# LSDOlab/femo_alpha

Measured on AMD Instinct MI355X. Metric: DOF/s (assembly+solve), forward solve of the RM shell; adjoint-gradient wallclock in adjoint_ms, higher is better.
Workload: dtype f64

## Files before the change

### femo_alpha_amd/csrc/femo_hip.hip

```cpp
#include "../../include/femo_hip.h"
#include "shell_device.h"
#include "frontal.h"
#include "sweeps_multi.h"
#include "shape_sens.h"
#include "residual_jvp.h"
#include "stress.h"
#include "stress_grad.h"
#include "stress_history.h"
#include "disp_history.h"
#include "ply_failure.h"
#include "field_jvp.h"
#include "layup.h"
#include "csr_map.h"
#include "hip_handles.h"

#include <hip/hip_runtime.h>

#include <algorithm>
#include <cmath>
#include <cstdio>
#include <cstdlib>
#include <cstring>
#include <string>
#include <utility>
// ... 5 lines not shown
constexpr int WIDE_CNT_DEFAULT = 512;

#define FEMO_VERSION 101

static std::string g_create_error;

struct femo_ctx {
    int device = 0;
    Stream stream;
    int krylov = 0;
    DevBuf<double> bi[5];
    int tab_nq = 0;
    double hK_mean = 0;
    DevBuf<double> mr_v, mr_y, mr_work, mr_scal;
    PinnedBuf<double> mr_scal_host;
    DevBuf<double> mr_io;
    long long opt_version = 0;
    Stream stream2;
    Event ev_la[2];
    Event ev_sp[2];
    Stream stream_g;
    Event ev_g[2];
    Stream stream_m;
    Event ev_da[2];
    Stream stream3;
    Stream stream_a;
    Event ev_a[3];
    Event ev_x[2];
    int nn = 0, nel = 0, nvc = 0, npc = 0, nP2 = 0, ndof_u = 0, ndof = 0, ld = 0;
    int nghost = 0;
// ... 102 lines not shown
        int fuse_rows_np = 2 * NBO;
        int sweep_graph = 0;
        int diag_v1_cnt = 512;
        int split_cnt = 0, split_groups = 2;
        int super_tiles = 0, super_tiles_min = 8;
        int diag_ahead = 0;
        int fused_schur = 1;
        int equilibrate = 0;
        int precond_nquad = 0;
        int grid_chunk = 32768;
        int wide_np = WIDE_NP_DEFAULT, wide_cnt = WIDE_CNT_DEFAULT;
        int strict = 1;
        int allow_pivot_repair = 0;
        int profile_verbose = 0;
        int big_tiles = 0, big_min_wg = 512;
        int strip_cnt = 0, strip_kmax = STRIP_KMAX, strip_depth = 1;
        int diag_v1 = 0;
        int swork_slots = 8192;
        int xinv_small_cnt = 32;
        int bnd_tiled_nb = 1 << 30;
        int sweep_butterfly = 3;
        int sweep_fuse = 0;
        int sweep_w = 0;
        int assemble_fc = 1;
        int sweep_ahead = 2;
        int apply_lanes = 0;
        int diag_t = 0;
        int multi_rhs = 1;
        int stale_factor = 0;
        double stale_rel = 2e-3;
        int sweep_read_mode = 0;
        int sh_levels_per_thread = 0;
        int sh_chunk = 0;
        int dh_chunk = 0;
// ... 626 lines not shown
            const dim3 grid(nt * (nt + 1) / 2, cnt);
            { ProfScope ps(c, 3);
              FOR_FRONT_CHUNKS(cnt, off, n)
                  hipLaunchKernelGGL(k_extend_gather, dim3(grid.x, n), dim3(256), 0, c->stream, fd, lev, off, mask, fused_schur ? 1 : 0); }
        }
        const bool wide = fr.h_level_wide[L];
        const int cnt_level = cnt, max_np_level = max_np;
        const int* lev_level = lev;
        const bool level_right = c->opt.trailing == 2 ? true : c->opt.trailing == 1 ? false : (cnt_level < c->opt.left_min || cnt_level > c->opt.left_max);
        const bool level_sp = level_right && SP_opt > NBO && cnt_level <= c->opt.super_panel_cnt && max_np_level > NBO;
        const bool level_la = level_right && !level_sp && cnt_level < c->opt.lookahead_cnt && c->opt.lookahead != 0;
        const bool split = wide && c->stream_g && cnt_level >= 2 && cnt_level <= c->opt.split_cnt && !level_la &&
                           !(level_sp && (c->opt.super_panel_ahead || c->opt.diag_ahead));
        const int ngroups = split ? std::max(2, std::min(cnt_level, c->opt.split_groups)) : 1;
        const int chunk_cap = split ? (cnt_level + ngroups - 1) / ngroups : wide ? cnt_level : std::min(cnt_level, fr.swork_slots);
        if (split) {
            HIPCHK(c, hipEventRecord(c->ev_g[0], c->stream));
            HIPCHK(c, hipStreamWaitEvent(c->stream_g, c->ev_g[0], 0));
        }
        for (int chunk_b = b; chunk_b < fr.h_level_off[L + 1]; chunk_b += chunk_cap) {
        hipStream_t st = (split && ((chunk_b - fr.h_level_off[L]) / chunk_cap) % 2 == 1) ? c->stream_g : c->stream;
        const int b = chunk_b, e = std::min(chunk_b + chunk_cap, fr.h_level_off[L + 1]);
        const int cnt = e - b;
        const int* lev = fr.level_nodes + b;
        int max_np = 0;
        for (int i = b; i < e; ++i) max_np = std::max(max_np, fr.h_npiv[fr.h_level_nodes[i]]);
        int max_nf = 0;
        for (int i = b; i < e; ++i) max_nf = std::max(max_nf, fr.h_nf[fr.h_level_nodes[i]]);
        int max_nb = 0;
        for (int i = b; i < e; ++i) max_nb = std::max(max_nb, fr.h_nf[fr.h_level_nodes[i]] - fr.h_npiv[fr.h_level_nodes[i]]);
        const bool right_looking = c->opt.trailing == 2 ? true : c->opt.trailing == 1 ? false : (cnt_level < c->opt.left_min || cnt_level > c->opt.left_max);
        const bool use_sp = right_looking && SP_opt > NBO && cnt_level <= c->opt.super_panel_cnt && max_np_level > NBO;
        const bool lookahead = right_looking && !use_sp && cnt_level < c->opt.lookahead_cnt && c->opt.lookahead != 0;
        bool bulk_pending = false;
        auto count_trailing = [&](int C0, int schur, int K0 = 0, int KW = NBO) {
            if (!fr.profile) return;
            double fl = 0, by = 0;
            for (int i = b; i < e; ++i) {
                const int t = fr.h_level_nodes[i], np = fr.h_npiv[t], nf = fr.h_nf[t];
                const TrailRange tr = trail_range(schur, C0, K0, KW, np, nf);
                const int kw = tr.kw, col_lo = tr.col_lo, col_hi = tr.col_hi;
                if (kw <= 0 || col_lo >= col_hi) continue;
                const double ncol = col_hi - col_lo;
                const double entries = ncol * nf - 0.5 * ncol * (col_lo + col_hi - 1.0);
                fl += 2.0 * kw * entries;
                by += 16.0 * entries + 8.0 * kw * (nf - col_lo);
            }
            fr.prof_flops[2] += fl; fr.prof_bytes[2] += by;
            fr.last_fl += fl; fr.last_by += by;
// ... 21 lines not shown
                if (kmax > 0 && kmax <= std::min(c->opt.strip_kmax, STRIP_KMAX)) {
                    const dim3 grid(gx, 1, n);
#define STRIP_LAUNCH(G_, KQ_, D_) hipLaunchKernelGGL((k_schur_strip<G_, KQ_, D_>), grid, dim3(256), 0, st, fd, lev, off, C0_, mode, K0_, KW_, mask)
#define STRIP_DEPTHS(G_, KQ_) do { if (c->opt.strip_depth <= 1) STRIP_LAUNCH(G_, KQ_, 1); else STRIP_LAUNCH(G_, KQ_, 2); } while (0)
                    if (gather) { if (kmax <= 64) STRIP_DEPTHS(true, 16); else if (kmax <= 112) STRIP_DEPTHS(true, 28); else if (kmax <= 128) STRIP_DEPTHS(true, 32); else STRIP_DEPTHS(true, 40); }
                    else        { if (kmax <= 64) STRIP_DEPTHS(false, 16); else if (kmax <= 128) STRIP_DEPTHS(false, 32); else STRIP_DEPTHS(false, 40); }
#undef STRIP_DEPTHS
#undef STRIP_LAUNCH
                    return;
                }
            }
            const int ntb = (ntr + 1) / 2;
            const long long big_wgs = (long long)ntb * (ntb + 1) / 2 * n;
            if (c->opt.big_tiles && big_wgs >= c->opt.big_min_wg) {
                const size_t shm = 4 * sizeof(double) * 16 * LSTRB;
                if (gather) hipLaunchKernelGGL(k_trailing_big<true>, dim3(ntb * (ntb + 1) / 2, 1, n), dim3(256), shm, st, fd, lev, off, C0_, mode, K0_, KW_, mask);
                else hipLaunchKernelGGL(k_trailing_big<false>, dim3(ntb * (ntb + 1) / 2, 1, n), dim3(256), shm, st, fd, lev, off, C0_, mode, K0_, KW_, mask);
            } else {
                const bool sup = c->opt.super_tiles && n < 256 && ntr >= c->opt.super_tiles_min;
                const int nst = (ntr + 3) / 4, nsup = nst * (nst + 1) / 2;
                const int gx = sup ? (nsup + 7) / 8 * 128 : ntr * (ntr + 1) / 2;
                if (gather) hipLaunchKernelGGL(k_trailing_mfma<true>, dim3(gx, 1, n), dim3(256), 0, st, fd, lev, off, C0_, mode, K0_, KW_, mask, 0, sup ? 1 : 0);
                else hipLaunchKernelGGL(k_trailing_mfma<false>, dim3(gx, 1, n), dim3(256), 0, st, fd, lev, off, C0_, mode, K0_, KW_, mask, 0, sup ? 1 : 0);
            }
        };
        auto narrow_slices = [&](int gx, int n, int K) {
            if (c->opt.narrow_split <= 1 || (long long)gx * n > c->opt.narrow_split_wg) return 1;
            return std::max(1, std::min(c->opt.narrow_split, K / 32));
        };
        auto launch_rows = [&](int ntiles, int off, int n, int C0_, const double* sw_, int tile_first, hipStream_t st) {
            if ((long long)ntiles * n <= c->opt.rows_fine_wg)
                hipLaunchKernelGGL(k_panel_rows_fine, dim3(4 * ntiles, n), dim3(256), 0, st, fd, lev, off, C0_, sw_, tile_first);
            else if ((long long)ntiles * n <= c->opt.rows_preload_wg)
                hipLaunchKernelGGL(k_panel_rows_preload, dim3(ntiles, n), dim3(256), PANEL_ROWS_PRELOAD_LDS, st, fd, lev, off, C0_, sw_, tile_first);
            else
                hipLaunchKernelGGL(k_panel_rows, dim3(ntiles, n), dim3(256), 0, st, fd, lev, off, C0_, sw_, tile_first);
        };
        auto count_panel = [&](int C0) {
// ... 20 lines not shown
            const int S0 = C0 / SP * SP;
            const int K0 = !right_looking ? 0 : sp_ahead ? std::max(0, S0 - SP) : S0;
            if (sp_ahead && C0 == S0 && sp_bulks >= 2)
                HIPCHK(c, hipStreamWaitEvent(st, c->ev_sp[sp_bulks & 1], 0));
            if (C0 > K0) {
                ProfScope ps(c, 2, st);
                count_trailing(C0, 0, K0);
                const int ntr = trail_tiles(C0, 0, K0);
                const bool gather_panel = fused_schur && K0 == 0;
                const int gx = diag_ahead ? std::min(DIAG_TILES, ntr * (NBO / TS)) : ntr * (NBO / TS);
                const bool fine = !diag_ahead && (C0 - K0) % 64 == 0 && (long long)gx * cnt <= c->opt.narrow_fine_wg;
                if (ntr > 0)
                FOR_FRONT_CHUNKS(cnt, off, n) {
                    if (fine) {
                        const int gx32 = 2 * ntr * (NBO / 32);
                        if (gather_panel) hipLaunchKernelGGL(k_trailing_fine<true>, dim3(gx32, 1, n), dim3(256), 0, st, fd, lev, off, C0, K0, mask, 0);
                        else hipLaunchKernelGGL(k_trailing_fine<false>, dim3(gx32, 1, n), dim3(256), 0, st, fd, lev, off, C0, K0, mask, 0);
                    } else if (gather_panel) hipLaunchKernelGGL(k_trailing_mfma<true>, dim3(gx, 1, n), dim3(256), 0, st, fd, lev, off, C0, 0, K0, NBO, mask, 0, 0);
                    else hipLaunchKernelGGL(k_trailing_mfma<false>, dim3(gx, narrow_slices(gx, n, C0 - K0), n), dim3(256), 0, st, fd, lev, off, C0, 0, K0, NBO, mask, 0, 0);
                }
            }
            count_panel(C0);
            { ProfScope ps(c, 1, st);
              const int* hn = fr.h_level_nodes.data() + b;
              auto first_above = [&](int thr) {
                  int lo = 0, hi = cnt;
                  while (lo < hi) { const int mid = (lo + hi) / 2; if (fr.h_npiv[hn[mid]] > thr) hi = mid; else lo = mid + 1; }
                  return lo;
              };
              int start = first_above(C0);
              for (int nb4 = 1; nb4 <= NBO / NB && start < cnt; ++nb4) {
                  int end = nb4 == NBO / NB ? cnt : first_above(C0 + NB * nb4);
                  int nblk = nb4;
                  if (cnt < 512) { end = cnt; nblk = std::min(NBO / NB, (fr.h_npiv[hn[cnt - 1]] - C0 + NB - 1) / NB); }
// ... 23 lines not shown
              } }
            int rows_below = 0;
            for (int i = b; i < e; ++i) {
                const int t = fr.h_level_nodes[i], np = fr.h_npiv[t];
                if (np > C0) rows_below = std::max(rows_below, fr.h_nf[t] - C0 - std::min(NBO, np - C0));
            }
            const int tiles = fuse_rows ? 0 : (rows_below + TS - 1) / TS;
            if (rest_pending) { HIPCHK(c, hipStreamWaitEvent(st, c->ev_da[1], 0)); rest_pending = false; }
            const bool ahead = diag_ahead && C0 + NBO < S0 + SP && C0 + NBO < max_np;
            const int tiles_main = ahead ? std::min(tiles, NEXT_ROW_TILES) : tiles;
            if (tiles_main > 0) {
                ProfScope ps(c, 0, st);
                FOR_FRONT_CHUNKS(cnt, off, n)
                    launch_rows(tiles_main, off, n, C0, sw, 0, st);
            }
            if (ahead) {
                HIPCHK(c, hipEventRecord(c->ev_da[0], st));
                HIPCHK(c, hipStreamWaitEvent(c->stream_m, c->ev_da[0], 0));
                if (tiles > tiles_main) {
                    ProfScope ps(c, 0, c->stream_m);
                    FOR_FRONT_CHUNKS(cnt, off, n)
                        launch_rows(tiles - tiles_main, off, n, C0, sw, tiles_main, c->stream_m);
                }
                const int C1 = C0 + NBO;
                const int gx = trail_tiles(C1, 0, K0) * (NBO / TS) - DIAG_TILES;
                if (gx > 0) {
                    ProfScope ps(c, 2, c->stream_m);
                    const bool gather_panel = fused_schur && K0 == 0;
                    FOR_FRONT_CHUNKS(cnt, off, n) {
                        if (gather_panel) hipLaunchKernelGGL(k_trailing_mfma<true>, dim3(gx, 1, n), dim3(256), 0, c->stream_m, fd, lev, off, C1, 0, K0, NBO, mask, DIAG_TILES, 0);
                        else hipLaunchKernelGGL(k_trailing_mfma<false>, dim3(gx, narrow_slices(gx, n, C1 - K0), n), dim3(256), 0, c->stream_m, fd, lev, off, C1, 0, K0, NBO, mask, DIAG_TILES, 0);
                    }
                }
                HIPCHK(c, hipEventRecord(c->ev_da[1], c->stream_m));
                rest_pending = true;
            }
            if (right_looking && SP > NBO) {
                if (C0 + NBO >= S0 + SP || C0 + NBO >= max_np) {
                    const int mode = sp_ahead ? 5 : 2;
                    const int ntr = trail_tiles(S0, mode, 0, SP);
                    if (ntr > 0) {
                        hipStream_t bs = sp_ahead ? c->stream2 : st;
                        if (sp_ahead) {
                            HIPCHK(c, hipEventRecord(c->ev_la[0], st));
                            HIPCHK(c, hipStreamWaitEvent(c->stream2, c->ev_la[0], 0));
                        }
// ... 4 lines not shown
                            HIPCHK(c, hipEventRecord(c->ev_sp[sp_bulks & 1], c->stream2));
                            ++sp_bulks;
                        }
                    }
                }
            } else if (right_looking && trail_tiles(C0, 2) > 0) {
                const int ntr = trail_tiles(C0, 2);
                if (!lookahead) {
                    ProfScope ps(c, 2, st);
                    count_trailing(C0, 2);
                    FOR_FRONT_CHUNKS(cnt, off, n) launch_tri(fused_schur && !left_level && C0 == 0, ntr, off, n, C0, 2, 0, NBO, st);
                } else {
                    if (bulk_pending) { HIPCHK(c, hipStreamWaitEvent(st, c->ev_la[1], 0)); bulk_pending = false; }
                    { ProfScope ps(c, 2, st);
                      count_trailing(C0, 3);
                      hipLaunchKernelGGL(k_trailing_mfma<false>, dim3(ntr * (NBO / TS), 1, cnt), dim3(256), 0, st, fd, lev, 0, C0, 3, 0, NBO, mask, 0, 0); }
                    const int ntb = trail_tiles(C0, 4);
                    if (ntb > 0) {
                        HIPCHK(c, hipEventRecord(c->ev_la[0], st));
                        HIPCHK(c, hipStreamWaitEvent(c->stream2, c->ev_la[0], 0));
                        { ProfScope ps(c, 2, c->stream2);
                          count_trailing(C0, 4);
                          hipLaunchKernelGGL(k_trailing_mfma<false>, dim3(ntb * (ntb + 1) / 2, 1, cnt), dim3(256), 0, c->stream2, fd, lev, 0, C0, 4, 0, NBO, mask, 0, 0); }
                        HIPCHK(c, hipEventRecord(c->ev_la[1], c->stream2));
                        bulk_pending = true;
                    }
                }
            }
        }
        if (bulk_pending) { HIPCHK(c, hipStreamWaitEvent(st, c->ev_la[1], 0)); bulk_pending = false; }
        if (rest_pending) { HIPCHK(c, hipStreamWaitEvent(st, c->ev_da[1], 0)); rest_pending = false; }
        if (sp_bulks > 0) HIPCHK(c, hipStreamWaitEvent(st, c->ev_sp[(sp_bulks - 1) & 1], 0));
        if (max_nb > 0 && !right_looking) {
            ProfScope ps(c, 2, st);
            count_trailing(0, 1);
            const int ntr = trail_tiles(0, 1);
            if (ntr > 0)
            FOR_FRONT_CHUNKS(cnt, off, n) launch_tri(fused_schur, ntr, off, n, 0, 1, 0, NBO, st);
        }
        }
        if (split) {
            HIPCHK(c, hipEventRecord(c->ev_g[1], c->stream_g));
            HIPCHK(c, hipStreamWaitEvent(c->stream, c->ev_g[1], 0));
        }
        const bool w_level = wide && fr.w_mode && fr.h_level_maxnb[L] > 0;
        if (wide && (max_np_level > NBO || w_level)) {
            const int max_np = max_np_level, cnt = cnt_level;
            const int* lev = lev_level;
            HIPCHK(c, hipEventRecord(c->ev_x[0], c->stream));
            HIPCHK(c, hipStreamWaitEvent(c->stream3, c->ev_x[0], 0));
            ProfScope ps(c, 6, c->stream3);
            const bool small_tiles = cnt <= c->opt.xinv_small_cnt;
            for (int bs = NBO; bs < max_np; bs *= 2) {
                const int npairs = (max_np + 2 * bs - 1) / (2 * bs);
                FOR_FRONT_CHUNKS(cnt, off, n) {
                    if (small_tiles) {
                        const dim3 grid(npairs * (bs / 64) * (bs / 32), n);
                        hipLaunchKernelGGL((k_xinv<0, 64, 32>), grid, dim3(256), 0, c->stream3, fd, lev, off, bs);
                        hipLaunchKernelGGL((k_xinv<1, 64, 32>), grid, dim3(256), 0, c->stream3, fd, lev, off, bs);
                    } else {
                        const dim3 grid(npairs * (bs / 128) * (bs / 64), n);
                        hipLaunchKernelGGL((k_xinv<0, 128, 64>), grid, dim3(256), 0, c->stream3, fd, lev, off, bs);
                        hipLaunchKernelGGL((k_xinv<1, 128, 64>), grid, dim3(256), 0, c->stream3, fd, lev, off, bs);
                    }
                }
            }
            if (w_level) {
                const int nrt = (fr.h_level_maxnb[L] + WT_M - 1) / WT_M;
                FOR_FRONT_CHUNKS(cnt, off, n) hipLaunchKernelGGL(k_w_inplace, dim3(nrt, n), dim3(256), 0, c->stream3, fd, lev, off);
            }
            x_pending = true;
            if (fr.profile) {
                HIPCHK(c, hipEventRecord(c->ev_x[1], c->stream3));
                HIPCHK(c, hipStreamWaitEvent(c->stream, c->ev_x[1], 0));
            }
        }
        HIPCHK(c, hipGetLastError());
        if (fr.ahead_vec && L + 1 == fr.nlevels - c->opt.sweep_ahead && l0 == 0 && l1 == fr.nlevels && !fr.profile) {
            HIPCHK(c, hipEventRecord(c->ev_a[0], c->stream));
            HIPCHK(c, hipStreamWaitEvent(c->stream_a, c->ev_a[0], 0));
// ... 412 lines not shown
    if (stale) {
        double* cur[6] = {c->h, c->E, c->nu, c->rho, c->has_uhat ? c->uhat : nullptr, c->laminate ? c->clt : nullptr};
        const int64_t len[6] = {c->nT, c->nT, c->nT, c->nT, 3 * (int64_t)c->nn, (int64_t)LAM_W * c->nel};
        for (int i = 0; i < 6 && stale; ++i) {
            if (!cur[i] && !c->fr.snap[i]) continue;
            if (!cur[i] || !c->fr.snap[i]) { stale = false; break; }
            HIPCHK(c, hipMemsetAsync(c->scal + 5, 0, 2 * sizeof(double), c->stream));
            hipLaunchKernelGGL(k_sq_change, dim3(red_grid(len[i])), dim3(256), 0, c->stream, (const double*)cur[i], (const double*)c->fr.snap[i], len[i], c->scal + 5);
            HIPCHK(c, hipMemcpyAsync(c->scal_host + 5, c->scal + 5, 2 * sizeof(double), hipMemcpyDeviceToHost, c->stream));
            HIPCHK(c, hipStreamSynchronize(c->stream));
            const double d2 = c->scal_host[5], r2 = i == 4 ? (double)c->nn * c->hK_mean * c->hK_mean : c->scal_host[6];
            if (!(d2 <= c->opt.stale_rel * c->opt.stale_rel * r2)) stale = false;
        }
    }
    int factor_state = stale ? 1 : 0;
    if (stale) { c->fr.t_assemble_ms = 0; c->fr.t_factor_ms = 0; }
    if (!c->fr.factored && !stale) {
        const bool ahead = zero_guess && c->opt.sweep_ahead > 0 && c->fr.nlevels > c->opt.sweep_ahead + 1 && !c->opt.equilibrate &&
                           c->opt.sweep_w == 0 && !c->opt.sweep_fuse;
        c->fr.ahead_levels = 0;
        if (ahead) {
            if (mask) hipLaunchKernelGGL(k_mask_zero, dim3(vg), dim3(256), 0, c->stream, b, mask, n);
            HIPCHK(c, hipMemcpyAsync(c->z, b, n * sizeof(double), hipMemcpyDeviceToDevice, c->stream));
            c->fr.ahead_vec = c->z;
        }
        const int rc = frontal_factorize(c);
        c->fr.ahead_vec = nullptr;
        if (rc) { c->fr.ahead_levels = 0; return rc; }
    }
    HIPCHK(c, hipEventRecord(c->ev[1], c->stream));
    auto dot = [&](const double* a, const double* bb, double* out) -> int {
        HIPCHK(c, hipMemsetAsync(c->scal + 7, 0, sizeof(double), c->stream));
        hipLaunchKernelGGL(k_dot, dim3(red_grid(n)), dim3(256), 0, c->stream, a, bb, n, c->scal + 7);
        HIPCHK(c, hipMemcpyAsync(c->scal_host + 7, c->scal + 7, sizeof(double), hipMemcpyDeviceToHost, c->stream));
        HIPCHK(c, hipStreamSynchronize(c->stream));
        *out = c->scal_host[7];
        return 0;
    };
    if (mask) hipLaunchKernelGGL(k_mask_zero, dim3(vg), dim3(256), 0, c->stream, b, mask, n);
    double bb = 0, rr = 0, pAp = 0;
    if (dot(b, b, &bb)) return 1;
    if (!std::isfinite(bb)) {
        if (c->fr.ahead_levels > 0) { HIPCHK(c, hipStreamWaitEvent(c->stream, c->ev_a[2], 0)); c->fr.ahead_levels = 0; }
        return fail(c, "PCG: the right-hand side is not finite (NaN or infinite b.b)");
    }
    if (zero_guess) {
        hipLaunchKernelGGL(k_fill, dim3(vg), dim3(256), 0, c->stream, x, 0.0, n);
        HIPCHK(c, hipMemcpyAsync(c->r, b, n * sizeof(double), hipMemcpyDeviceToDevice, c->stream));
    } else {
        if (mask) hipLaunchKernelGGL(k_mask_zero, dim3(vg), dim3(256), 0, c->stream, x, mask, n);
        hipLaunchKernelGGL(k_fill, dim3(vg), dim3(256), 0, c->stream, c->Ap, 0.0, n);
        if (op_apply(c, x, c->Ap, nullptr, nullptr, nullptr, true, c->op_aK, c->op_aM)) return 1;
        HIPCHK(c, hipMemcpyAsync(c->r, b, n * sizeof(double), hipMemcpyDeviceToDevice, c->stream));
        hipLaunchKernelGGL(k_axpby, dim3(vg), dim3(256), 0, c->stream, c->r, -1.0, c->Ap, 1.0, n);
        if (mask) hipLaunchKernelGGL(k_mask_zero, dim3(vg), dim3(256), 0, c->stream, c->r, mask, n);
    }
// ... 1084 lines not shown
    else if (k == "fused_schur") o.fused_schur = v != 0;
    else if (k == "precond_nquad") { if (v != 0 && (v < 2 || v > 6)) return fail(c, "precond_nquad: 0 (the operator's rule) or 2..6"); o.precond_nquad = v; operator_changed(c); }
    else if (k == "equilibrate") { if (v < 0 || v > 2) return fail(c, "equilibrate: 0 off, 1 diag^-1/2, 2 nearest powers of two"); o.equilibrate = v; operator_changed(c); }
    else if (k == "grid_chunk") { if (v < 1 || v > 65535) return fail(c, "grid_chunk must be in 1..65535"); o.grid_chunk = v; }
    else if (k == "wide_np" || k == "wide_cnt") {
        if (c->fr.ready) return fail(c, "wide_np / wide_cnt shape the plan: set them before femo_set_frontal_plan");
        if (v < 0) return fail(c, "negative threshold");
        (k == "wide_np" ? o.wide_np : o.wide_cnt) = v;
    }
    else if (k == "strict") o.strict = v != 0;
    else if (k == "allow_pivot_repair") o.allow_pivot_repair = v != 0;
    else if (k == "stress_regularization") { if (value < 0) return fail(c, "stress_regularization: a coefficient >= 0 (the reference's is 0.5e3)"); c->stress_reg = value; }
    else if (k == "profile_verbose") o.profile_verbose = v != 0;
    else if (k == "big_tiles") o.big_tiles = v != 0;
    else if (k == "big_min_wg") o.big_min_wg = v;
    else if (k == "strip_cnt") o.strip_cnt = v;
    else if (k == "strip_kmax") o.strip_kmax = v;
    else if (k == "strip_depth") { if (v < 1 || v > 2) return fail(c, "strip_depth: 1..2 blocks of look-ahead"); o.strip_depth = v; }
    else if (k == "diag_v1") { if (v < 0 || v > 3) return fail(c, "diag_v1: 0 auto, 1 round-2 kernel, 2 overlapped kernel, 3 the rule before the LDS diet"); o.diag_v1 = v; }
    else if (k == "profile") c->fr.profile = v != 0;
    else if (k == "bnd_tiled_nb") o.bnd_tiled_nb = v;
    else if (k == "sweep_butterfly") o.sweep_butterfly = v;
    else if (k == "sweep_fuse") o.sweep_fuse = v != 0;
    else if (k == "assemble_fc") { if (v < 0 || v > 2) return fail(c, "assemble_fc: 0 never, 1 where it pays, 2 always"); o.assemble_fc = v; }
    else if (k == "sweep_w") { if ((v != 0) != (o.sweep_w != 0)) { o.sweep_w = v != 0; operator_changed(c); } }
    else if (k == "multi_rhs") { o.multi_rhs = v != 0; }
    else if (k == "diag_t") { o.diag_t = v; }
    else if (k == "apply_lanes") { if (v != 0 && v != 4 && v != 5) return fail(c, "apply_lanes: 0 or 4 (a quad of lanes per element), or 5"); o.apply_lanes = v; }
    else if (k == "sweep_ahead") { if (v < 0) return fail(c, "sweep_ahead: number of top levels left to the solve (0: off)"); o.sweep_ahead = v; }
    else if (k == "stale_rel") { if (!(value >= 0)) return fail(c, "stale_rel: a relative change >= 0"); o.stale_rel = value; }
    else if (k == "stress_history_levels_per_thread") { if (v < 0) return fail(c, "stress_history_levels_per_thread: >= 0 (0: automatic)"); o.sh_levels_per_thread = v; }
    else if (k == "stress_history_chunk") { if (v < 0) return fail(c, "stress_history_chunk: >= 0 levels (0: automatic)"); o.sh_chunk = v; }
    else if (k == "disp_history_chunk") { if (v < 0) return fail(c, "disp_history_chunk: >= 0 levels (0: automatic)"); o.dh_chunk = v; }
    else if (k == "stale_factor") { if (v < 0) return fail(c, "stale_factor: PCG iterations a kept factor is given before the factorisation is refreshed (0: never keep)"); o.stale_factor = v; }
    else if (k == "sweep_read_mode") { if (v < 0 || v > 2) return fail(c, "sweep_read_mode: 0 returning atomic, 1 agent-scope load, 2 plain load (experiment)"); o.sweep_read_mode = v; }
    else if (k == "swork_slots") { if (c->fr.ready || v < 1) return fail(c, "swork_slots >= 1, before femo_set_frontal_plan"); o.swork_slots = v; }
    else if (k == "xinv_small_cnt") o.xinv_small_cnt = v;
    else return fail(c, "unknown option '" + k + "'");
    return 0;
}

int femo_set_krylov(femo_ctx* c, int method) {
    if (method != 0 && method != 1) return fail(c, "Krylov method must be 0 (conjugate gradients) or 1 (BiCGStab)");
    c->krylov = method;
    return 0;
}

int femo_solve_state(femo_ctx* c, int zero_guess, int32_t* iters, double* relres) {
    HIPCHK(c, hipSetDevice(c->device));
    if (load_vector_dev(c, c->b)) return 1;
    return solve_dispatch(c, c->b, c->w, zero_guess != 0, iters, relres);
}
// ... 298 lines not shown
    hipMemcpyAsync(c->lam, lambda, (size_t)c->ndof * sizeof(double), hipMemcpyHostToDevice, c->stream);
    if (int rc = dRdarg_T_dev(c, arg ? arg : "", c->lam, 1.0, d, n)) return rc;
    HIPCHK(c, hipStreamSynchronize(c->stream));
    HIPCHK(c, hipMemcpy(out, d, (size_t)n * sizeof(double), hipMemcpyDeviceToHost));
    return 0;
}

int femo_total_gradient(femo_ctx* c, const char* functional, const char* arg, double* out, int64_t n, int32_t* iters,
                        double* relres) {
    HIPCHK(c, hipSetDevice(c->device));
    const std::string fn(functional ? functional : ""), a(arg ? arg : "");
    if (fn == "ply_failure") {
        if (ply_need_table(c, "ply_failure")) return 2;
        if (a == "uhat") return fail(c, "ply_failure: the shape derivative (uhat) of this output is not provided");
    }
    DevBuf<double> d;
    HIPCHK(c, d.alloc(std::max<int64_t>(n, 1)));
    int rc = dfunctional_dev(c, fn, "disp_solid", c->b, c->ndof);
    if (!rc) rc = solve_dispatch(c, c->b, c->lam, true, iters, relres);
    if (!rc) rc = dfunctional_dev(c, fn, a, d, n);
    if (!rc) rc = dRdarg_T_dev(c, a, c->lam, -1.0, d, n);
    if (rc) return rc;
    HIPCHK(c, hipStreamSynchronize(c->stream));
    HIPCHK(c, hipMemcpy(out, d, (size_t)n * sizeof(double), hipMemcpyDeviceToHost));
    return 0;
}


static bool multi_sweeps_apply(const femo_ctx* c) {
    return c->precond == 2 && c->krylov == 0 && c->fr.ready && c->opt.sweep_w == 0 && !c->opt.equilibrate && c->opt.multi_rhs != 0;
}

// ... 2075 lines not shown
```

### femo_alpha_amd/csrc/frontal.h

```cpp
#pragma once
#include "shell_device.h"

namespace femo {

constexpr int NB = 32;
constexpr int TS = 64;
constexpr int NBO = 128;
constexpr int SPD = 128;

struct FrontDev {
    int ntree;
    const int* nf;
    const int* npiv;
    const long long* poff;
    const long long* soff;
    const long long* doff;
    const int* dofs;
    const int* upmap;
    const int* parent;
    const int* child[2];
    const int* cinv[2];
    const long long* linvoff;
    const long long* xoff;
    double* P;
// ... 1315 lines not shown
struct TrailRange { int kc0, kw, col_lo, col_hi; };
__device__ __host__ inline TrailRange trail_range(int schur, int C0, int K0, int KW, int np, int nf) {
    TrailRange r{0, 0, 0, 0};
    if (schur != 1 && C0 >= np) return r;
    r.kc0 = schur >= 2 ? C0 : (schur ? 0 : K0);
    r.kw = schur >= 2 ? (KW < np - C0 ? KW : np - C0) : (schur ? np : C0 - K0);
    const int split = ((C0 + r.kw) & ~1) + NBO;
    r.col_lo = schur >= 2 ? (schur == 4 ? split : schur == 5 ? (C0 + 2 * KW < np ? C0 + 2 * KW : np) : C0 + r.kw) : (schur ? np : C0);
    r.col_hi = schur == 0 ? (C0 + NBO < np ? C0 + NBO : np) : schur == 3 ? (split < nf ? split : nf) : nf;
    return r;
}

template <bool GATHER>
__global__ void __launch_bounds__(256, 4)
k_trailing_mfma(FrontDev fd, const int* __restrict__ level_nodes, int first, int C0, int schur, int K0, int KW,
                const unsigned char* __restrict__ mask, int bx_first, int tile_map) {
    int bxv = blockIdx.x, zv = blockIdx.z;
    {
        const int G = gridDim.x, n = gridDim.z;
        if (n >= 256 && (n & 7) == 0) {
            const int flat = bxv + G * zv, x = flat & 7, q = flat >> 3;
            zv = (q / G) * 8 + x; bxv = q % G;
        }
    }
    bxv += bx_first;
    const int t = level_nodes[first + zv];
    const int np = fd.npiv[t];
    const int nf = fd.nf[t];
    const TrailRange tr = trail_range(schur, C0, K0, KW, np, nf);
    int kc0 = tr.kc0, kw = tr.kw;
    const int col_lo = tr.col_lo, col_hi = tr.col_hi;
// ... 58 lines not shown
    };
    if (kw >= KC) fetch(base); else fetch_tail(base, kw);
    base += stage_bytes;
    mfma_d4 acc[2][2];
#pragma unroll
    for (int a = 0; a < 2; ++a)
#pragma unroll
        for (int b = 0; b < 2; ++b) acc[a][b] = (mfma_d4){0.0, 0.0, 0.0, 0.0};
#pragma unroll
    for (int q = 0; q < 2; ++q) {
        *reinterpret_cast<d2*>(&si[0][cg + 8 * q][2 * rp]) = pi[q];
        *reinterpret_cast<d2*>(&sj[0][cg + 8 * q][2 * rp]) = pj[q];
    }
    __syncthreads();
    int cur = 0;
    const bool idle_quarter = ri == cj && wr + 31 < wc;
    for (int k0 = 0; k0 < kw; k0 += KC) {
        const int left = kw - k0 - KC;
        if (left > 0) {
            if (left >= KC) fetch(base); else fetch_tail(base, left);
            base += stage_bytes;
        }
        if (!idle_quarter) {
#pragma unroll
        for (int kk = 0; kk < KC; kk += 4) {
            const double a0 = sj[cur][kk + l4][wc + l15], a1 = sj[cur][kk + l4][wc + 16 + l15];
            const double b0 = si[cur][kk + l4][wr + l15], b1 = si[cur][kk + l4][wr + 16 + l15];
            acc[0][0] = __builtin_amdgcn_mfma_f64_16x16x4f64(a0, b0, acc[0][0], 0, 0, 0);
            acc[0][1] = __builtin_amdgcn_mfma_f64_16x16x4f64(a0, b1, acc[0][1], 0, 0, 0);
            acc[1][0] = __builtin_amdgcn_mfma_f64_16x16x4f64(a1, b0, acc[1][0], 0, 0, 0);
            acc[1][1] = __builtin_amdgcn_mfma_f64_16x16x4f64(a1, b1, acc[1][1], 0, 0, 0);
// ... 126 lines not shown
    }
#pragma unroll
    for (int a = 0; a < 2; ++a)
#pragma unroll
        for (int b = 0; b < 2; ++b)
#pragma unroll
            for (int reg = 0; reg < 4; ++reg) {
                const int cc = cj + wc + 16 * a + l4 + 4 * reg;
                const int r = ri + wr + 16 * b + l15;
                if (cok[a][reg] && r < nf && r >= cc) col_ptr(a, reg)[r] = cv[a][b][reg] - acc[a][b][reg];
            }
}

template <bool GATHER>
__global__ void __launch_bounds__(256, 2)
k_trailing_fine(FrontDev fd, const int* __restrict__ level_nodes, int first, int C0, int K0, const unsigned char* __restrict__ mask, int bx_first) {
    const int t = level_nodes[first + blockIdx.z];
    const int np = fd.npiv[t];
    const int nf = fd.nf[t];
    const TrailRange tr = trail_range(0, C0, K0, NBO, np, nf);
    const int kc0 = tr.kc0, kw = tr.kw, col_lo = tr.col_lo, col_hi = tr.col_hi;
    if (kw <= 0) return;
    constexpr int FT = 32;
    const int bxv = (int)blockIdx.x + bx_first;
    const int by = bxv & 3, bx = bxv >> 2;
    const int cj = (col_lo & ~1) + by * FT;
    if (cj >= col_hi) return;
    const int ri = cj + bx * FT;
    if (ri >= nf) return;
    const FrontView fv = front_view(fd, t);
    const int tid = threadIdx.x, lane = tid & 63, wv = tid >> 6;
    const int wr = (wv & 1) * 16, wc = (wv >> 1) * 16;
    const int l15 = lane & 15, l4 = lane >> 4;
    const int ldp = ldp_of(nf);
    const double* pa = fv.P + min(cj + wc + l15, nf - 1) + (size_t)ldp * (kc0 + l4);
    const double* pb = fv.P + min(ri + wr + l15, nf - 1) + (size_t)ldp * (kc0 + l4);
    const size_t kstep = (size_t)ldp * 4;
    constexpr int KB = 32, NS = KB / 4;
    double a0[NS], b0[NS], a1[NS], b1[NS];
    mfma_d4 acc = (mfma_d4){0.0, 0.0, 0.0, 0.0};
    const int nbatch = kw / KB;
#pragma unroll
    for (int s_ = 0; s_ < NS; ++s_) { a0[s_] = pa[kstep * s_]; b0[s_] = pb[kstep * s_]; }
    for (int bt = 0; bt < nbatch; bt += 2) {
        const bool more1 = bt + 1 < nbatch, more2 = bt + 2 < nbatch;
        if (more1) {
#pragma unroll
// ... 220 lines not shown
        if (cb_lo + d < cb_hi) request(cb_lo + d, g[d], okm[d]);
    }
    for (int cb = cb_lo; cb < cb_hi; cb += NSET) {
#pragma unroll
        for (int u = 0; u < NSET; ++u)
            if (cb + u < cb_hi) stage(cb + u, g[u], okm[u], g[(u + DEPTH) % NSET], okm[(u + DEPTH) % NSET], pa[u], pa[(u + 1) % NSET]);
    }
}

constexpr int TSB = 128;
constexpr int LSTRB = TSB + 16;

template <bool GATHER>
__global__ void __launch_bounds__(256, 2)
k_trailing_big(FrontDev fd, const int* __restrict__ level_nodes, int first, int C0, int schur, int K0, int KW,
               const unsigned char* __restrict__ mask) {
    const int t = level_nodes[first + blockIdx.z];
    const int np = fd.npiv[t];
    const int nf = fd.nf[t];
    const TrailRange tr = trail_range(schur, C0, K0, KW, np, nf);
    const int kc0 = tr.kc0, kw = tr.kw, col_lo = tr.col_lo, col_hi = tr.col_hi;
    if (kw <= 0) return;
    const int lin = blockIdx.x;
    int ti = (int)((sqrt(8.0 * lin + 1.0) - 1.0) * 0.5);
    while ((ti + 1) * (ti + 2) / 2 <= lin) ++ti;
    while (ti * (ti + 1) / 2 > lin) --ti;
    const int by = lin - ti * (ti + 1) / 2, bx = ti - by;
    const int cj = (col_lo & ~1) + by * TSB;
    if (cj >= col_hi) return;
    const int ri = cj + bx * TSB;
    if (ri >= nf) return;
// ... 40 lines not shown
        for (int q = 0; q < 4; ++q) {
            *reinterpret_cast<d2*>(&si[buf][cg + 4 * q][2 * rp]) = pi[q];
            *reinterpret_cast<d2*>(&sj[buf][cg + 4 * q][2 * rp]) = pj[q];
        }
    };
    if (kw >= KC) fetch(base); else fetch_tail(base, kw);
    base += stage_bytes;
    mfma_d4 acc[4][4];
#pragma unroll
    for (int a = 0; a < 4; ++a)
#pragma unroll
        for (int b = 0; b < 4; ++b) acc[a][b] = (mfma_d4){0.0, 0.0, 0.0, 0.0};
    stash(0);
    __syncthreads();
    int cur = 0;
    for (int k0 = 0; k0 < kw; k0 += KC) {
        const int left = kw - k0 - KC;
        if (left > 0) {
            if (left >= KC) fetch(base); else fetch_tail(base, left);
            base += stage_bytes;
        }
#pragma unroll
        for (int kk = 0; kk < KC; kk += 4) {
            double av[4], bv[4];
#pragma unroll
            for (int a = 0; a < 4; ++a) av[a] = sj[cur][kk + l4][wc + 16 * a + l15];
#pragma unroll
            for (int b = 0; b < 4; ++b) bv[b] = si[cur][kk + l4][wr + 16 * b + l15];
#pragma unroll
            for (int a = 0; a < 4; ++a)
#pragma unroll
                for (int b = 0; b < 4; ++b) acc[a][b] = __builtin_amdgcn_mfma_f64_16x16x4f64(av[a], bv[b], acc[a][b], 0, 0, 0);
        }
        if (left > 0) stash(cur ^ 1);
        __syncthreads();
        cur ^= 1;
    }
    const long long dp = fd.doff[t];
    int rr[2][4];
    const double* Sc[2] = {nullptr, nullptr};
    int npc[2] = {0, 0}, nbc[2] = {0, 0}, chv[2] = {-1, -1};
    if (GATHER) {
#pragma unroll
        for (int sd = 0; sd < 2; ++sd) {
            const int ch = fd.child[sd][t];
            const int chs = ch >= 0 ? ch : t;
            chv[sd] = ch;
            npc[sd] = fd.npiv[chs]; nbc[sd] = fd.nf[chs] - npc[sd];
            Sc[sd] = fd.S + fd.soff[chs];
#pragma unroll
            for (int b = 0; b < 4; ++b) {
                const int r = ri + wr + 16 * b + l15;
// ... 664 lines not shown
        for (int k = 0; k < 32; ++k) {
            const int c = c0 + 32 * wv + k;
            const bool ca = c < np && ra < np && ra >= c, cbb = c < np && rb < np && rb >= c;
            p[k] = (ca ? a0[k] : 0.0) * x0 + (cbb ? a1[k] : 0.0) * x1;
        }
        int colw;
        const double sum = wave_sum_cols<32>(p, lane, colw);
        const int c = c0 + 32 * wv + colw;
        if (!(lane & 1) && c < np) sweep_add(&xv[gd[c]], sum);
        sweep_signal(nullptr, xfin);
    }
}

template <int PHASE, int TM, int TN>
__global__ void __launch_bounds__(256)
k_xinv(FrontDev fd, const int* __restrict__ level_nodes, int first, int bs) {
    const int t = level_nodes[first + blockIdx.y];
    const int np = fd.npiv[t];
    const int rts = bs / TM, cts = bs / TN;
    int lin = blockIdx.x;
    const int ct = lin % cts; lin /= cts;
    const int rt = lin % rts;
    const int pair = lin / rts;
    const int a0 = 2 * pair * bs, b0 = a0 + bs;
    if (b0 >= np) return;
    const int mB = min(bs, np - b0);
    const int r0 = rt * TM;
    if (r0 >= mB) return;
    const int c0 = ct * TN;
    const int nf = fd.nf[t], ldx = ldx_of(np);
    const double* F = fd.P + fd.poff[t];
    double* X = fd.X + fd.xoff[t];
    double* T = fd.Xtmp + fd.xoff[t];
    const int k_lo = PHASE == 0 ? (c0 & ~15) : 0;
    const int k_hi = PHASE == 0 ? bs : min(mB, r0 + TM);
    constexpr int KC = 16, SA = TM + 16, SB = TN + 16;
    constexpr int GA = 256 / TM, QA = KC / GA;
    constexpr int QB = TN / 16;
// ... 156 lines not shown
```

Baseline: 62.49 million.

## Skip idle trailing-update waves, pipeline X inversion, hoist b·b dot, reuse gradient buffer

Adds a trail_blocks option, on by default, that lets waves in the trailing-update kernels skip MFMA work or exit when none of their 16x16 output blocks store anything. Adds an optional xinv_pipe_cnt mode, off by default, that launches X-inverse pairs on a side stream as soon as enough panel columns are finished. Also moves the b·b reduction and its host copy ahead of factorization, so the PCG start no longer needs a separate sync after factorizing. A persistent buffer now replaces a per-call allocation in the total-gradient path. Together these aim to cut wasted triangular-tile work and sync and allocation overhead, at the cost of extra per-wave branching.

Result: no change. 62.47 million (-0.0%).

```diff
diff --git a/femo_alpha_amd/csrc/femo_hip.hip b/femo_alpha_amd/csrc/femo_hip.hip
--- a/femo_alpha_amd/csrc/femo_hip.hip
+++ b/femo_alpha_amd/csrc/femo_hip.hip
@@ -43,6 +43,7 @@
     double hK_mean = 0;
     DevBuf<double> mr_v, mr_y, mr_work, mr_scal;
     PinnedBuf<double> mr_scal_host;
+    DevBuf<double> tg_out;
     DevBuf<double> mr_io;
     long long opt_version = 0;
     Stream stream2;
@@ -175,10 +176,12 @@
         int allow_pivot_repair = 0;
         int profile_verbose = 0;
         int big_tiles = 0, big_min_wg = 512;
+        int trail_blocks = 1;
         int strip_cnt = 0, strip_kmax = STRIP_KMAX, strip_depth = 1;
         int diag_v1 = 0;
         int swork_slots = 8192;
         int xinv_small_cnt = 32;
+        int xinv_pipe_cnt = 0;
         int bnd_tiled_nb = 1 << 30;
         int sweep_butterfly = 3;
         int sweep_fuse = 0;
@@ -835,6 +838,22 @@
                            !(level_sp && (c->opt.super_panel_ahead || c->opt.diag_ahead));
         const int ngroups = split ? std::max(2, std::min(cnt_level, c->opt.split_groups)) : 1;
         const int chunk_cap = split ? (cnt_level + ngroups - 1) / ngroups : wide ? cnt_level : std::min(cnt_level, fr.swork_slots);
+        auto launch_xinv = [&](int bs, int p0, int np_) {
+            const bool small_tiles = cnt_level <= c->opt.xinv_small_cnt;
+            FOR_FRONT_CHUNKS(cnt_level, off, n) {
+                if (small_tiles) {
+                    const dim3 grid(np_ * (bs / 64) * (bs / 32), n);
+                    hipLaunchKernelGGL((k_xinv<0, 64, 32>), grid, dim3(256), 0, c->stream3, fd, lev_level, off, bs, p0);
+                    hipLaunchKernelGGL((k_xinv<1, 64, 32>), grid, dim3(256), 0, c->stream3, fd, lev_level, off, bs, p0);
+                } else {
+                    const dim3 grid(np_ * (bs / 128) * (bs / 64), n);
+                    hipLaunchKernelGGL((k_xinv<0, 128, 64>), grid, dim3(256), 0, c->stream3, fd, lev_level, off, bs, p0);
+                    hipLaunchKernelGGL((k_xinv<1, 128, 64>), grid, dim3(256), 0, c->stream3, fd, lev_level, off, bs, p0);
+                }
+            }
+        };
+        int xp_done[32] = {0};
+        const bool xpipe = wide && !fr.profile && !split && max_np_level > NBO && c->opt.xinv_pipe_cnt > 0 && cnt_level <= c->opt.xinv_pipe_cnt;
         if (split) {
             HIPCHK(c, hipEventRecord(c->ev_g[0], c->stream));
             HIPCHK(c, hipStreamWaitEvent(c->stream_g, c->ev_g[0], 0));
@@ -854,6 +873,7 @@
         const bool use_sp = right_looking && SP_opt > NBO && cnt_level <= c->opt.super_panel_cnt && max_np_level > NBO;
         const bool lookahead = right_looking && !use_sp && cnt_level < c->opt.lookahead_cnt && c->opt.lookahead != 0;
         bool bulk_pending = false;
+        const int tblk = c->opt.trail_blocks;
         auto count_trailing = [&](int C0, int schur, int K0 = 0, int KW = NBO) {
             if (!fr.profile) return;
             double fl = 0, by = 0;
@@ -905,14 +925,14 @@
             const long long big_wgs = (long long)ntb * (ntb + 1) / 2 * n;
             if (c->opt.big_tiles && big_wgs >= c->opt.big_min_wg) {
                 const size_t shm = 4 * sizeof(double) * 16 * LSTRB;
-                if (gather) hipLaunchKernelGGL(k_trailing_big<true>, dim3(ntb * (ntb + 1) / 2, 1, n), dim3(256), shm, st, fd, lev, off, C0_, mode, K0_, KW_, mask);
-                else hipLaunchKernelGGL(k_trailing_big<false>, dim3(ntb * (ntb + 1) / 2, 1, n), dim3(256), shm, st, fd, lev, off, C0_, mode, K0_, KW_, mask);
+                if (gather) hipLaunchKernelGGL(k_trailing_big<true>, dim3(ntb * (ntb + 1) / 2, 1, n), dim3(256), shm, st, fd, lev, off, C0_, mode, K0_, KW_, mask, tblk);
+                else hipLaunchKernelGGL(k_trailing_big<false>, dim3(ntb * (ntb + 1) / 2, 1, n), dim3(256), shm, st, fd, lev, off, C0_, mode, K0_, KW_, mask, tblk);
             } else {
                 const bool sup = c->opt.super_tiles && n < 256 && ntr >= c->opt.super_tiles_min;
                 const int nst = (ntr + 3) / 4, nsup = nst * (nst + 1) / 2;
                 const int gx = sup ? (nsup + 7) / 8 * 128 : ntr * (ntr + 1) / 2;
-                if (gather) hipLaunchKernelGGL(k_trailing_mfma<true>, dim3(gx, 1, n), dim3(256), 0, st, fd, lev, off, C0_, mode, K0_, KW_, mask, 0, sup ? 1 : 0);
-                else hipLaunchKernelGGL(k_trailing_mfma<false>, dim3(gx, 1, n), dim3(256), 0, st, fd, lev, off, C0_, mode, K0_, KW_, mask, 0, sup ? 1 : 0);
+                if (gather) hipLaunchKernelGGL(k_trailing_mfma<true>, dim3(gx, 1, n), dim3(256), 0, st, fd, lev, off, C0_, mode, K0_, KW_, mask, 0, sup ? 1 : 0, tblk);
+                else hipLaunchKernelGGL(k_trailing_mfma<false>, dim3(gx, 1, n), dim3(256), 0, st, fd, lev, off, C0_, mode, K0_, KW_, mask, 0, sup ? 1 : 0, tblk);
             }
         };
         auto narrow_slices = [&](int gx, int n, int K) {
@@ -963,10 +983,10 @@
                 FOR_FRONT_CHUNKS(cnt, off, n) {
                     if (fine) {
                         const int gx32 = 2 * ntr * (NBO / 32);
-                        if (gather_panel) hipLaunchKernelGGL(k_trailing_fine<true>, dim3(gx32, 1, n), dim3(256), 0, st, fd, lev, off, C0, K0, mask, 0);
-                        else hipLaunchKernelGGL(k_trailing_fine<false>, dim3(gx32, 1, n), dim3(256), 0, st, fd, lev, off, C0, K0, mask, 0);
-                    } else if (gather_panel) hipLaunchKernelGGL(k_trailing_mfma<true>, dim3(gx, 1, n), dim3(256), 0, st, fd, lev, off, C0, 0, K0, NBO, mask, 0, 0);
-                    else hipLaunchKernelGGL(k_trailing_mfma<false>, dim3(gx, narrow_slices(gx, n, C0 - K0), n), dim3(256), 0, st, fd, lev, off, C0, 0, K0, NBO, mask, 0, 0);
+                        if (gather_panel) hipLaunchKernelGGL(k_trailing_fine<true>, dim3(gx32, 1, n), dim3(256), 0, st, fd, lev, off, C0, K0, mask, 0, tblk);
+                        else hipLaunchKernelGGL(k_trailing_fine<false>, dim3(gx32, 1, n), dim3(256), 0, st, fd, lev, off, C0, K0, mask, 0, tblk);
+                    } else if (gather_panel) hipLaunchKernelGGL(k_trailing_mfma<true>, dim3(gx, 1, n), dim3(256), 0, st, fd, lev, off, C0, 0, K0, NBO, mask, 0, 0, tblk);
+                    else hipLaunchKernelGGL(k_trailing_mfma<false>, dim3(gx, narrow_slices(gx, n, C0 - K0), n), dim3(256), 0, st, fd, lev, off, C0, 0, K0, NBO, mask, 0, 0, tblk);
                 }
             }
             count_panel(C0);
@@ -1020,6 +1040,23 @@
                 FOR_FRONT_CHUNKS(cnt, off, n)
                     launch_rows(tiles_main, off, n, C0, sw, 0, st);
             }
+            if (xpipe && !diag_ahead) {
+                const int done_cols = C0 + NBO, all_cols = (max_np + NBO - 1) / NBO * NBO;
+                bool joined = false;
+                for (int bs = NBO, ib = 0; bs < max_np; bs *= 2, ++ib) {
+                    const int npairs = (max_np + 2 * bs - 1) / (2 * bs);
+                    int ready = xp_done[ib];
+                    while (ready < npairs && std::min((2 * ready + 2) * bs, all_cols) <= done_cols) ++ready;
+                    if (ready == xp_done[ib]) continue;
+                    if (!joined) {
+                        HIPCHK(c, hipEventRecord(c->ev_x[0], st));
+                        HIPCHK(c, hipStreamWaitEvent(c->stream3, c->ev_x[0], 0));
+                        joined = true;
+                    }
+                    launch_xinv(bs, xp_done[ib], ready - xp_done[ib]);
+                    xp_done[ib] = ready;
+                }
+            }
             if (ahead) {
                 HIPCHK(c, hipEventRecord(c->ev_da[0], st));
                 HIPCHK(c, hipStreamWaitEvent(c->stream_m, c->ev_da[0], 0));
@@ -1034,8 +1071,8 @@
                     ProfScope ps(c, 2, c->stream_m);
                     const bool gather_panel = fused_schur && K0 == 0;
                     FOR_FRONT_CHUNKS(cnt, off, n) {
-                        if (gather_panel) hipLaunchKernelGGL(k_trailing_mfma<true>, dim3(gx, 1, n), dim3(256), 0, c->stream_m, fd, lev, off, C1, 0, K0, NBO, mask, DIAG_TILES, 0);
-                        else hipLaunchKernelGGL(k_trailing_mfma<false>, dim3(gx, narrow_slices(gx, n, C1 - K0), n), dim3(256), 0, c->stream_m, fd, lev, off, C1, 0, K0, NBO, mask, DIAG_TILES, 0);
+                        if (gather_panel) hipLaunchKernelGGL(k_trailing_mfma<true>, dim3(gx, 1, n), dim3(256), 0, c->stream_m, fd, lev, off, C1, 0, K0, NBO, mask, DIAG_TILES, 0, tblk);
+                        else hipLaunchKernelGGL(k_trailing_mfma<false>, dim3(gx, narrow_slices(gx, n, C1 - K0), n), dim3(256), 0, c->stream_m, fd, lev, off, C1, 0, K0, NBO, mask, DIAG_TILES, 0, tblk);
                     }
                 }
                 HIPCHK(c, hipEventRecord(c->ev_da[1], c->stream_m));
@@ -1070,14 +1107,14 @@
                     if (bulk_pending) { HIPCHK(c, hipStreamWaitEvent(st, c->ev_la[1], 0)); bulk_pending = false; }
                     { ProfScope ps(c, 2, st);
                       count_trailing(C0, 3);
-                      hipLaunchKernelGGL(k_trailing_mfma<false>, dim3(ntr * (NBO / TS), 1, cnt), dim3(256), 0, st, fd, lev, 0, C0, 3, 0, NBO, mask, 0, 0); }
+                      hipLaunchKernelGGL(k_trailing_mfma<false>, dim3(ntr * (NBO / TS), 1, cnt), dim3(256), 0, st, fd, lev, 0, C0, 3, 0, NBO, mask, 0, 0, tblk); }
                     const int ntb = trail_tiles(C0, 4);
                     if (ntb > 0) {
                         HIPCHK(c, hipEventRecord(c->ev_la[0], st));
                         HIPCHK(c, hipStreamWaitEvent(c->stream2, c->ev_la[0], 0));
                         { ProfScope ps(c, 2, c->stream2);
                           count_trailing(C0, 4);
-                          hipLaunchKernelGGL(k_trailing_mfma<false>, dim3(ntb * (ntb + 1) / 2, 1, cnt), dim3(256), 0, c->stream2, fd, lev, 0, C0, 4, 0, NBO, mask, 0, 0); }
+                          hipLaunchKernelGGL(k_trailing_mfma<false>, dim3(ntb * (ntb + 1) / 2, 1, cnt), dim3(256), 0, c->stream2, fd, lev, 0, C0, 4, 0, NBO, mask, 0, 0, tblk); }
                         HIPCHK(c, hipEventRecord(c->ev_la[1], c->stream2));
                         bulk_pending = true;
                     }
@@ -1106,20 +1143,9 @@
             HIPCHK(c, hipEventRecord(c->ev_x[0], c->stream));
             HIPCHK(c, hipStreamWaitEvent(c->stream3, c->ev_x[0], 0));
             ProfScope ps(c, 6, c->stream3);
-            const bool small_tiles = cnt <= c->opt.xinv_small_cnt;
-            for (int bs = NBO; bs < max_np; bs *= 2) {
+            for (int bs = NBO, ib = 0; bs < max_np; bs *= 2, ++ib) {
                 const int npairs = (max_np + 2 * bs - 1) / (2 * bs);
-                FOR_FRONT_CHUNKS(cnt, off, n) {
-                    if (small_tiles) {
-                        const dim3 grid(npairs * (bs / 64) * (bs / 32), n);
-                        hipLaunchKernelGGL((k_xinv<0, 64, 32>), grid, dim3(256), 0, c->stream3, fd, lev, off, bs);
-                        hipLaunchKernelGGL((k_xinv<1, 64, 32>), grid, dim3(256), 0, c->stream3, fd, lev, off, bs);
-                    } else {
-                        const dim3 grid(npairs * (bs / 128) * (bs / 64), n);
-                        hipLaunchKernelGGL((k_xinv<0, 128, 64>), grid, dim3(256), 0, c->stream3, fd, lev, off, bs);
-                        hipLaunchKernelGGL((k_xinv<1, 128, 64>), grid, dim3(256), 0, c->stream3, fd, lev, off, bs);
-                    }
-                }
+                if (xp_done[ib] < npairs) launch_xinv(bs, xp_done[ib], npairs - xp_done[ib]);
             }
             if (w_level) {
                 const int nrt = (fr.h_level_maxnb[L] + WT_M - 1) / WT_M;
@@ -1562,6 +1588,7 @@
         }
     }
     int factor_state = stale ? 1 : 0;
+    bool bb_early = false;
     if (stale) { c->fr.t_assemble_ms = 0; c->fr.t_factor_ms = 0; }
     if (!c->fr.factored && !stale) {
         const bool ahead = zero_guess && c->opt.sweep_ahead > 0 && c->fr.nlevels > c->opt.sweep_ahead + 1 && !c->opt.equilibrate &&
@@ -1572,9 +1599,14 @@
             HIPCHK(c, hipMemcpyAsync(c->z, b, n * sizeof(double), hipMemcpyDeviceToDevice, c->stream));
             c->fr.ahead_vec = c->z;
         }
+        if (mask && !ahead) hipLaunchKernelGGL(k_mask_zero, dim3(vg), dim3(256), 0, c->stream, b, mask, n);
+        HIPCHK(c, hipMemsetAsync(c->scal + 7, 0, sizeof(double), c->stream));
+        hipLaunchKernelGGL(k_dot, dim3(red_grid(n)), dim3(256), 0, c->stream, (const double*)b, (const double*)b, n, c->scal + 7);
+        HIPCHK(c, hipMemcpyAsync(c->scal_host + 7, c->scal + 7, sizeof(double), hipMemcpyDeviceToHost, c->stream));
         const int rc = frontal_factorize(c);
         c->fr.ahead_vec = nullptr;
         if (rc) { c->fr.ahead_levels = 0; return rc; }
+        bb_early = true;
     }
     HIPCHK(c, hipEventRecord(c->ev[1], c->stream));
     auto dot = [&](const double* a, const double* bb, double* out) -> int {
@@ -1585,9 +1617,12 @@
         *out = c->scal_host[7];
         return 0;
     };
-    if (mask) hipLaunchKernelGGL(k_mask_zero, dim3(vg), dim3(256), 0, c->stream, b, mask, n);
     double bb = 0, rr = 0, pAp = 0;
-    if (dot(b, b, &bb)) return 1;
+    if (bb_early) bb = c->scal_host[7];
+    else {
+        if (mask) hipLaunchKernelGGL(k_mask_zero, dim3(vg), dim3(256), 0, c->stream, b, mask, n);
+        if (dot(b, b, &bb)) return 1;
+    }
     if (!std::isfinite(bb)) {
         if (c->fr.ahead_levels > 0) { HIPCHK(c, hipStreamWaitEvent(c->stream, c->ev_a[2], 0)); c->fr.ahead_levels = 0; }
         return fail(c, "PCG: the right-hand side is not finite (NaN or infinite b.b)");
@@ -2702,6 +2737,7 @@
     else if (k == "profile_verbose") o.profile_verbose = v != 0;
     else if (k == "big_tiles") o.big_tiles = v != 0;
     else if (k == "big_min_wg") o.big_min_wg = v;
+    else if (k == "trail_blocks") { if (v != 0 && v != 1) return fail(c, "trail_blocks: 0 whole tiles, 1 skip the waves whose 16 x 16 blocks store nothing"); o.trail_blocks = v; }
     else if (k == "strip_cnt") o.strip_cnt = v;
     else if (k == "strip_kmax") o.strip_kmax = v;
     else if (k == "strip_depth") { if (v < 1 || v > 2) return fail(c, "strip_depth: 1..2 blocks of look-ahead"); o.strip_depth = v; }
@@ -2724,6 +2760,7 @@
     else if (k == "sweep_read_mode") { if (v < 0 || v > 2) return fail(c, "sweep_read_mode: 0 returning atomic, 1 agent-scope load, 2 plain load (experiment)"); o.sweep_read_mode = v; }
     else if (k == "swork_slots") { if (c->fr.ready || v < 1) return fail(c, "swork_slots >= 1, before femo_set_frontal_plan"); o.swork_slots = v; }
     else if (k == "xinv_small_cnt") o.xinv_small_cnt = v;
+    else if (k == "xinv_pipe_cnt") { if (v < 0) return fail(c, "xinv_pipe_cnt: wide levels of at most this many fronts form X beside their chain of panels (0: off)"); o.xinv_pipe_cnt = v; }
     else return fail(c, "unknown option '" + k + "'");
     return 0;
 }
@@ -3052,8 +3089,8 @@
         if (ply_need_table(c, "ply_failure")) return 2;
         if (a == "uhat") return fail(c, "ply_failure: the shape derivative (uhat) of this output is not provided");
     }
-    DevBuf<double> d;
-    HIPCHK(c, d.alloc(std::max<int64_t>(n, 1)));
+    HIPCHK(c, c->tg_out.grow(std::max<int64_t>(n, 1)));
+    double* d = c->tg_out;
     int rc = dfunctional_dev(c, fn, "disp_solid", c->b, c->ndof);
     if (!rc) rc = solve_dispatch(c, c->b, c->lam, true, iters, relres);
     if (!rc) rc = dfunctional_dev(c, fn, a, d, n);
diff --git a/femo_alpha_amd/csrc/frontal.h b/femo_alpha_amd/csrc/frontal.h
--- a/femo_alpha_amd/csrc/frontal.h
+++ b/femo_alpha_amd/csrc/frontal.h
@@ -1353,7 +1353,7 @@
 template <bool GATHER>
 __global__ void __launch_bounds__(256, 4)
 k_trailing_mfma(FrontDev fd, const int* __restrict__ level_nodes, int first, int C0, int schur, int K0, int KW,
-                const unsigned char* __restrict__ mask, int bx_first, int tile_map) {
+                const unsigned char* __restrict__ mask, int bx_first, int tile_map, int blocks) {
     int bxv = blockIdx.x, zv = blockIdx.z;
     {
         const int G = gridDim.x, n = gridDim.z;
@@ -1442,7 +1442,20 @@
     }
     __syncthreads();
     int cur = 0;
-    const bool idle_quarter = ri == cj && wr + 31 < wc;
+    bool idle_quarter = ri == cj && wr + 31 < wc;
+    if (blocks) {
+        const int wvu = __builtin_amdgcn_readfirstlane(wv);
+        const int wru = (wvu & 1) * 32, wcu = (wvu >> 1) * 32;
+        bool live = false;
+#pragma unroll
+        for (int a = 0; a < 2; ++a)
+#pragma unroll
+            for (int b = 0; b < 2; ++b) {
+                const int c0 = cj + wcu + 16 * a, r0 = ri + wru + 16 * b;
+                live = live || (r0 < nf && c0 < col_hi && c0 + 15 >= col_lo && r0 + 15 >= c0);
+            }
+        idle_quarter = !live;
+    }
     for (int k0 = 0; k0 < kw; k0 += KC) {
         const int left = kw - k0 - KC;
         if (left > 0) {
@@ -1599,7 +1612,8 @@
 
 template <bool GATHER>
 __global__ void __launch_bounds__(256, 2)
-k_trailing_fine(FrontDev fd, const int* __restrict__ level_nodes, int first, int C0, int K0, const unsigned char* __restrict__ mask, int bx_first) {
+k_trailing_fine(FrontDev fd, const int* __restrict__ level_nodes, int first, int C0, int K0, const unsigned char* __restrict__ mask, int bx_first,
+                int blocks) {
     const int t = level_nodes[first + blockIdx.z];
     const int np = fd.npiv[t];
     const int nf = fd.nf[t];
@@ -1616,6 +1630,11 @@
     const FrontView fv = front_view(fd, t);
     const int tid = threadIdx.x, lane = tid & 63, wv = tid >> 6;
     const int wr = (wv & 1) * 16, wc = (wv >> 1) * 16;
+    if (blocks) {
+        const int wvu = __builtin_amdgcn_readfirstlane(wv);
+        const int r0 = ri + (wvu & 1) * 16, c0 = cj + (wvu >> 1) * 16;
+        if (!(r0 < nf && c0 < col_hi && c0 + 15 >= col_lo && r0 + 15 >= c0)) return;
+    }
     const int l15 = lane & 15, l4 = lane >> 4;
     const int ldp = ldp_of(nf);
     const double* pa = fv.P + min(cj + wc + l15, nf - 1) + (size_t)ldp * (kc0 + l4);
@@ -1866,7 +1885,7 @@
 template <bool GATHER>
 __global__ void __launch_bounds__(256, 2)
 k_trailing_big(FrontDev fd, const int* __restrict__ level_nodes, int first, int C0, int schur, int K0, int KW,
-               const unsigned char* __restrict__ mask) {
+               const unsigned char* __restrict__ mask, int blocks) {
     const int t = level_nodes[first + blockIdx.z];
     const int np = fd.npiv[t];
     const int nf = fd.nf[t];
@@ -1937,12 +1956,27 @@
     stash(0);
     __syncthreads();
     int cur = 0;
+    bool idle_quarter = false;
+    if (blocks) {
+        const int wvu = __builtin_amdgcn_readfirstlane(wv);
+        const int wru = (wvu & 1) * 64, wcu = (wvu >> 1) * 64;
+        bool live = false;
+#pragma unroll
+        for (int a = 0; a < 4; ++a)
+#pragma unroll
+            for (int b = 0; b < 4; ++b) {
+                const int c0 = cj + wcu + 16 * a, r0 = ri + wru + 16 * b;
+                live = live || (r0 < nf && c0 < col_hi && c0 + 15 >= col_lo && r0 + 15 >= c0);
+            }
+        idle_quarter = !live;
+    }
     for (int k0 = 0; k0 < kw; k0 += KC) {
         const int left = kw - k0 - KC;
         if (left > 0) {
             if (left >= KC) fetch(base); else fetch_tail(base, left);
             base += stage_bytes;
         }
+        if (!idle_quarter) {
 #pragma unroll
         for (int kk = 0; kk < KC; kk += 4) {
             double av[4], bv[4];
@@ -1955,10 +1989,12 @@
 #pragma unroll
                 for (int b = 0; b < 4; ++b) acc[a][b] = __builtin_amdgcn_mfma_f64_16x16x4f64(av[a], bv[b], acc[a][b], 0, 0, 0);
         }
+        }
         if (left > 0) stash(cur ^ 1);
         __syncthreads();
         cur ^= 1;
     }
+    if (idle_quarter) return;
     const long long dp = fd.doff[t];
     int rr[2][4];
     const double* Sc[2] = {nullptr, nullptr};
@@ -2653,14 +2689,14 @@
 
 template <int PHASE, int TM, int TN>
 __global__ void __launch_bounds__(256)
-k_xinv(FrontDev fd, const int* __restrict__ level_nodes, int first, int bs) {
+k_xinv(FrontDev fd, const int* __restrict__ level_nodes, int first, int bs, int pair0) {
     const int t = level_nodes[first + blockIdx.y];
     const int np = fd.npiv[t];
     const int rts = bs / TM, cts = bs / TN;
     int lin = blockIdx.x;
     const int ct = lin % cts; lin /= cts;
     const int rt = lin % rts;
-    const int pair = lin / rts;
+    const int pair = pair0 + lin / rts;
     const int a0 = 2 * pair * bs, b0 = a0 + bs;
     if (b0 >= np) return;
     const int mB = min(bs, np - b0);
```
